# fbcotter/pytorch_wavelets

Measured on AMD Instinct MI355X. Metric: Mpixels/s fwd+inv DWT J=3 db4, Nx3x512x512 fp32; % HBM roofline, higher is better.
Workload: dtype f32; 1 GPU; DWTForward+DWTInverse J=3 db4 symmetric, 128x3x512x512 fp32 per GPU (BASELINE configs[1]); global_batch=128, parallelism=batch-sharded x1, no data-path collective, step=forward + inverse

## Files before the change

### pytorch_wavelets_amd/csrc/wl_api.inc

```
#include "../../include/wavelets_hip.h"
#include "wl_common.h"
#include "wl_api_common.h"
#include "wl_dt_api.h"
#include <string.h>
#include "wl_dwt_kernels.h"
#include "wl_dwt_tile.h"
#include "wl_dwt_tile_syn.h"
#include "wl_dwt_direct.h"
#include "wl_nonsep.h"
#include "wl_dwt_small.h"
#include "wl_filt1d.h"
#include "wl_swt2d.h"
#include "wl_iswt2d.h"
#include "wl_dwt3d.h"
#include "wl_dtcwt_kernels.h"
#include "wl_dtcwt_tile.h"
#include "wl_dtcwt_rot.h"
#include "wl_dtcwt_small.h"

template <typename T>
struct WlAfb2dTile {
    typedef WlAfb2dArgs<T> Args;
    static const int kThreads = 256;
    static const int kMinWaves = 1;
    static WL_DEV void run(const Args& a, const WlCtx& ctx) { wl_afb2d_tile_body<T>(a, ctx); }
};
template <typename T>
struct WlSfb2dTile {
    typedef WlSfb2dArgs<T> Args;
    static const int kThreads = 256;
    static const int kMinWaves = 1;
    static WL_DEV void run(const Args& a, const WlCtx& ctx) { wl_sfb2d_tile_body<T>(a, ctx); }
};

extern "C" int wl_version(void) { return 220; }
extern "C" const char* wl_backend(void) { return WL_BACKEND_NAME; }
extern "C" int wl_dwt_coeff_len(int n, int L, int mode) { return wl_coeff_len(n, L, mode); }

struct WlOptions {
    int generic_only;
    int no_stream;
    int scat_stream;
    WlOptions() {
        const char* v = getenv("WL_GENERIC_ONLY");
        generic_only = (v && *v) ? atoi(v) : 0;
        no_stream = 0;
        scat_stream = 0;
    }
};
static WlOptions& wl_options() { static WlOptions o; return o; }
extern "C" int wl_set_option(const char* name, int value) {
    if (!name) return WL_ERR_SHAPE;
    if (!strcmp(name, "generic_only")) { wl_options().generic_only = value; return 0; }
    if (!strcmp(name, "no_stream")) { wl_options().no_stream = value; return 0; }
    if (!strcmp(name, "scat_stream")) { wl_options().scat_stream = value; return 0; }
    return WL_ERR_UNSUPPORTED;
}
extern "C" int wl_get_option(const char* name) {
    if (!name) return WL_ERR_SHAPE;
    if (!strcmp(name, "generic_only")) return wl_options().generic_only;
    if (!strcmp(name, "no_stream")) return wl_options().no_stream;
    if (!strcmp(name, "scat_stream")) return wl_options().scat_stream;
    return WL_ERR_UNSUPPORTED;
}
extern "C" const char* wl_last_kernel(void) { return wl_last_kernel_name(); }
extern "C" const char* wl_kernel_history(int back) { return wl_kernel_history_name(back); }
extern "C" long long wl_launch_count(void) { return wl_launch_count_value(); }
extern "C" long long wl_last_grid(void) { return wl_last_grid_value(); }
int wl_streaming_off() { return wl_options().no_stream || wl_options().generic_only; }

template <typename T>
static int wl_afb2d_generic(const WlAfbReq& r) {
    typedef typename WlAcc<T>::type A;
    const int H = r.H, W = r.W, Lw = r.Lw, Lh = r.Lh, mode = r.mode;
    WlAfb2dArgs<T> a;
    a.x = (const T*)r.x; a.ll = (T*)r.ll; a.highs = (T*)r.highs;
    a.h_w_lo = (const A*)r.taps.w_lo; a.h_w_hi = (const A*)r.taps.w_hi; a.h_h_lo = (const A*)r.taps.h_lo; a.h_h_hi = (const A*)r.taps.h_hi;
    a.NC = r.planes; a.H = H; a.W = W;
    a.x_ps = r.x_ps; a.ll_ps = r.ll_ps; a.x_rs = r.x_rs; a.ll_rs = r.ll_rs;
    a.Kh = wl_dwt_coeff_len(H, Lh, mode); a.Kw = wl_dwt_coeff_len(W, Lw, mode);
    a.Lw = Lw; a.Lh = Lh;
    a.basew = wl_afb_base(W, Lw, mode); a.baseh = wl_afb_base(H, Lh, mode);
    a.extw = a.exth = wl_mode_to_ext(mode);
    int TH = 16, TW = 64;
    if (a.Kw <= 32) TW = 32;
    if (a.Kh <= 8) TH = 8;
    for (;;) {
        a.TH = TH; a.TW = TW;
        a.nrows = 2 * TH + Lh - 2; a.ncols = 2 * TW + Lw - 2;
        a.spitch = a.ncols | 1;
        if (wl_afb2d_tile_lds(a) <= 64 * 1024 || (TH <= 4 && TW <= 16)) break;
        if (TW > 16) TW /= 2; else TH /= 2;
    }
    a.tiles_x = wl_cdiv(a.Kw, TW); a.tiles_y = wl_cdiv(a.Kh, TH);
    return wl_launch<WlAfb2dTile<T> >(a, r.planes * a.tiles_x * a.tiles_y, wl_afb2d_tile_lds(a), r.stream);
}


template <typename T, int LT, int TH = 16, int TW = 64, int SH = 0, int V4 = 0>
static int wl_afb_tile_launch(const WlAfbReq& r) {
    typedef WlAfbTile<T, LT, TH, TW, SH, V4> K;
    const int64_t planes = r.planes;
// ... 1013 lines not shown
```

### pytorch_wavelets_amd/csrc/wl_api_common.h

```cpp
#pragma once
#include <stdlib.h>
#include "../../include/wavelets_hip.h"
#include "wl_common.h"
#include "wl_lattice.h"

static int wl_mode_to_ext(int mode) {
    switch (mode) {
        case 0: return WL_EXT_ZERO;
        case 1: return WL_EXT_SYM;
        case 2: return WL_EXT_PER;
        case 4: return WL_EXT_REFL;
        case 6: return WL_EXT_PERIODIC;
        default: return -1;
    }
}

static inline int wl_coeff_len(int n, int L, int mode) { return mode == 2 ? (n + 1) / 2 : (n + L - 1) / 2; }

static int wl_afb_base(int n, int L, int mode) {
    if (mode == 2) return L / 2 - L + 1;
    const int K = (n + L - 1) / 2;
    const int p = 2 * (K - 1) - n + L;
    return -(p / 2);
}

struct WlBanks { const void* w_lo; const void* w_hi; const void* h_lo; const void* h_hi; };
struct WlAfbReq {
    const void* x; int64_t x_ps; int x_rs;
    void* ll; int64_t ll_ps; int ll_rs; void* highs;
    int64_t planes; int H, W;
    WlBanks taps; int Lw, Lh, mode;
    int policy; float* scratch; int* tstate; void* stream;
};
struct WlSfbReq {
    const void* ll; int64_t ll_ps; int ll_rs; const void* highs; void* y;
    int64_t planes; int Kh, Kw, OH, OW;
    WlBanks taps; int Lw, Lh, mode;
// ... 61 lines not shown
```

### pytorch_wavelets_amd/csrc/wl_dwt_rows.h

```cpp
#pragma once
#include "wl_common.h"

#define WL_ROWS_MAXLEV 3
#ifndef WL_ROWS_WAVES
#define WL_ROWS_WAVES 12
#endif
#ifndef WL_ROWS_LOADERS
#define WL_ROWS_LOADERS 2
#endif
#define WL_ROWS_MAXHB 768
#ifndef WL_ROWS_ABLATE
#define WL_ROWS_ABLATE 0
#endif
#if (WL_ROWS_ABLATE & 8) && defined(__HIPCC__)
#define WL_TICK() __builtin_readcyclecounter()
#else
#define WL_TICK() 0ull
#endif
#ifndef WL_ROWS_DEPTH
#define WL_ROWS_DEPTH 3
#endif

#if defined(__HIPCC__)
WL_DEV void wl_pk_fma_x(wl_v2& acc, wl_v2 tap, wl_v2 s) {
// ... 33 lines not shown
    int nwaves;
    unsigned ring_magic;
    int ring_rows;
};

struct WlRowsSeg {
    int nhb;
    int f0[WL_ROWS_MAXLEV];
    int fend[WL_ROWS_MAXLEV];
    int own_lo[WL_ROWS_MAXLEV];
    int own_hi[WL_ROWS_MAXLEV];
    unsigned sched[WL_ROWS_MAXHB / 4];
};

template <typename T>
struct WlRowsArgs {
    const T* x;
    T* ll;
    T* yh[WL_ROWS_MAXLEV];
    const float* h_w_lo;
    const float* h_w_hi;
    const float* h_h_lo;
    const float* h_h_hi;
    int64_t NC, x_ps, ll_ps;
    int x_rs, ll_rs;
    int nlev, ext, base;
    int nwhole;
    int zero_off;
    int lds_bytes;
    signed char role_level[WL_ROWS_WAVES];
    short role_col0[WL_ROWS_WAVES];
    signed char role_sub[WL_ROWS_WAVES];
    int pp, lds_plane;
    WlRowsLevel g[WL_ROWS_MAXLEV];
    WlRowsSeg seg[3];
    int guard;
    const float* lat;
};

struct WlRowsSched {
    int fed[WL_ROWS_MAXLEV];
    WL_HD void init(const WlRowsSeg& sg) { for (int j = 0; j < WL_ROWS_MAXLEV; ++j) fed[j] = sg.f0[j]; }
    static WL_HD int src_row(int e, int Hs, int ext) { return ext == WL_EXT_PER ? e : wl_ext1(e, Hs, ext); }
    WL_HD int avail(const WlRowsSeg& sg, int j, int LT) const {
        const int warm = (LT - 2) / 2;
        return fed[j] - sg.f0[j] > warm ? fed[j] - warm : sg.f0[j];
    }
    template <typename A> WL_HD int feeds_now(const A& a, const WlRowsSeg& sg, int j, int LT) const {
        const int left = sg.fend[j] - fed[j];
        if (j == 0) return left > 2 ? 2 : left;
        const int av = avail(sg, j - 1, LT);
        const int Hs = a.g[j].Hs;
        const int e = a.base + 2 * fed[j];
        const bool ok0 = left > 0 && src_row(e, Hs, a.ext) < av && src_row(e + 1, Hs, a.ext) < av;
        const bool ok1 = left > 1 && src_row(e + 2, Hs, a.ext) < av && src_row(e + 3, Hs, a.ext) < av;
        return ok0 ? (ok1 ? 2 : 1) : 0;
    }
};

#ifndef WL_ROWS_SAME_MIN
#define WL_ROWS_SAME_MIN 10
#endif
WL_HD int wl_ring_slot(int r, int rows, unsigned magic) {
    const unsigned u = (unsigned)(r + (rows << 6));
    const unsigned q = (unsigned)(((unsigned long long)u * magic) >> 32);
    const int sl = (int)(u - q * (unsigned)rows);
// ... 8 lines not shown
    static const int kThreads = 64 * WL_ROWS_WAVES;
    static const int kMinWaves = 6;
    static const int LROWS = 4 / WL_ROWS_LOADERS;
    static const int NL = LROWS * PPR;
    static const int WARM = (LT - 2) / 2;
    static const int NSLOT = D + 1;
    static const int SZ = (int)sizeof(T);
    static_assert((D - 1) * NL < 64, "prefetch distance exceeds the vmcnt range");

    static WL_DEV void loader(const Args& a, const WlRowsSeg& sg, const WlCtx& ctx, int64_t plane, int lane, int lidx) {
        const WlRowsLevel& g = a.g[0];
        const char* xp = reinterpret_cast<const char*>(a.x + (size_t)plane * a.x_ps);
        const int row_bytes = g.Ws * SZ;
        const int row_stride = a.x_rs * SZ;
        const int nhb0 = (sg.fend[0] - sg.f0[0] + 1) / 2;
        const int e_last = a.base + 2 * sg.fend[0] - 1;
        const int ring = g.ring_off, pitch = g.ring_pitch, pad = g.pad, Hs = g.Hs, ext = a.ext;
        const int base = a.base + 2 * sg.f0[0];
        const int rfirst = lidx * LROWS;
        const int NH = g.hl + g.hr;
        int hdst[2], hsrc[2];
#pragma unroll
        for (int u = 0; u < 2; ++u) {
            const int it = lane + 64 * u;
            hdst[u] = hsrc[u] = -1;
            if ((ext != WL_EXT_ZERO || row_bytes % 16 != 0) && it < LROWS * NH) {
                const int r = rfirst + it / NH, c = it % NH;
                const int e = c < g.hl ? c - g.hl : g.Ws + (c - g.hl);
                const int s = wl_ext(e, g.Ws, ext);
                hdst[u] = r * pitch + pad + e * SZ;
                hsrc[u] = s < 0 ? -1 : r * pitch + pad + s * SZ;
            }
        }
        auto issue = [&](int h) {
            const int slot = ring + (h % NSLOT) * 4 * pitch + pad;
#pragma unroll
            for (int rr = 0; rr < LROWS; ++rr) {
                const int r = rfirst + rr;
                int e = base + 4 * h + r;
                e = e < e_last ? e : e_last;
                int src = e;
                if ((unsigned)e >= (unsigned)Hs) {
                    src = wl_ext(e, Hs, ext);
                    src = src < 0 ? 0 : src;
                }
                const char* grow = xp + (size_t)src * row_stride;
#pragma unroll
                for (int p = 0; p < PPR; ++p) {
                    const int byte = (p * 64 + lane) * 16;
                    if (!(WL_ROWS_ABLATE & 2)) wl_dma16(ctx, (unsigned)(slot + r * pitch + p * 1024), grow + byte, byte < row_bytes);
                }
            }
        };
        for (int h = 0; h < D; ++h) issue(h);
        unsigned long long tw = 0, tb = 0, ti = 0;
        for (int hb = 0; hb < sg.nhb; ++hb) {
            const unsigned long long c0 = WL_TICK();
            if (hb < nhb0) {
                if (!(WL_ROWS_ABLATE & 2)) wl_wait_vm<(D - 1) * NL>();
                char* slot = ctx.smem + ring + (hb % NSLOT) * 4 * pitch;
#pragma unroll
                for (int u = 0; u < 2; ++u)
                    if (hdst[u] >= 0) *reinterpret_cast<T*>(slot + hdst[u]) = hsrc[u] < 0 ? (T)0 : *reinterpret_cast<const T*>(slot + hsrc[u]);
            }
            const unsigned long long c1 = WL_TICK();
            ctx.sync();
            const unsigned long long c2 = WL_TICK();
            if (hb < nhb0) issue(hb + D);
            const unsigned long long c3 = WL_TICK();
            tw += c1 - c0; tb += c2 - c1; ti += c3 - c2;
        }
        wl_wait_vm<0>();
        if ((WL_ROWS_ABLATE & 8) && lane == 0) {
            T* o = a.ll + (size_t)plane * a.ll_ps;
            o[8] = (T)(float)(tw >> 6); o[9] = (T)(float)(tb >> 6); o[10] = (T)(float)(ti >> 6);
        }
    }

    struct Lane {
        wl_v2 win[LAT ? (KL > 1 ? KL - 1 : 1) : LT];
        unsigned ob;
        int off;
        int ndst, hx0, hx1;
    };
    struct Role {
        wl_v2 tw[LAT ? KL : LT], th[SAME ? 1 : LT];
        wl_v2 lt[LAT ? KL : 1];
        WL_DEV wl_v2 colt(int t) const { return SAME ? tw[LAT ? 0 : t] : th[SAME ? 0 : t]; }
        char* hp0; char* hp1; char* hp2; char* llp;
        unsigned rowb, llrowb, kb;
        int nring, npitch, rmask;
        unsigned nmagic;
        bool last, halo;
    };

    static WL_DEV void load_rows(const Lane& L, const char* smem, int row0, int row1, wl_v2 (&s0)[NP], wl_v2 (&s1)[NP]) {
        const char* p0 = smem + (row0 + L.off);
        const char* p1 = smem + (row1 + L.off);
        if (SZ == 4) {
#pragma unroll
            for (int u = 0; u < NP; ++u) {
// ... 189 lines not shown
        R.llp = reinterpret_cast<char*>(a.ll + (size_t)plane * a.ll_ps);
        R.rowb = (unsigned)g.Kw * SZ; R.llrowb = (unsigned)a.ll_rs * SZ; R.kb = (unsigned)k * SZ;
        const WlRowsLevel& gn = a.g[j + 1 < WL_ROWS_MAXLEV ? j + 1 : j];
        R.nring = gn.ring_off; R.npitch = gn.ring_pitch;
        R.rmask = NP2 ? gn.ring_rows : gn.ring_rows - 1;
        R.nmagic = gn.ring_magic;
        Lane L;
#pragma unroll
        for (int t = 0; t < (LAT ? (KL > 1 ? KL - 1 : 1) : LT); ++t) L.win[t] = wl_v2{0.f, 0.f};
        L.ob = (unsigned)sg.f0[j] * R.rowb + (unsigned)k * SZ;
        L.off = g.pad + (2 * (active ? k : 0) + a.base - ODD) * SZ;
        L.ndst = gn.pad + k * SZ; L.hx0 = L.hx1 = -1;
        if (!R.last && active && a.ext != WL_EXT_ZERO) {
            for (int c = 0; c < gn.hl + gn.hr; ++c) {
                const int e = c < gn.hl ? c - gn.hl : gn.Ws + (c - gn.hl);
                if (wl_ext(e, gn.Ws, a.ext) == k) {
                    if (e < 0) L.hx0 = gn.pad + e * SZ; else L.hx1 = gn.pad + e * SZ;
                }
            }
        }
        R.halo = !R.last && a.ext != WL_EXT_ZERO && (col0 <= gn.hl + 1 || col0 + 63 >= gn.Ws - gn.hr - 2);
        if (R.last) main_loop<j, true, false>(a, sg, ctx, plane, L, R, active, k);
        else if (R.halo) main_loop<j, false, true>(a, sg, ctx, plane, L, R, active, k);
        else main_loop<j, false, false>(a, sg, ctx, plane, L, R, active, k);
    }

    template <int j, bool LAST, bool HALO>
    static WL_DEV void main_loop(const Args& a, const WlRowsSeg& sg, const WlCtx& ctx, int64_t plane, Lane& L, const Role& R,
                                 bool active, int k) {
        const WlRowsLevel& g = a.g[j];
        char* const smem = ctx.smem;
        const int rmask = NP2 ? g.ring_rows : g.ring_rows - 1, zrow = a.zero_off, ring = g.ring_off, pitch = g.ring_pitch, Hs = g.Hs;
        const bool zmode = a.ext == WL_EXT_ZERO, per = a.ext == WL_EXT_PER;
        auto rows_of = [&](int f, int hb, int i, int& r0, int& r1) {
            const int e = a.base + 2 * f;
            if (j == 0) {
                r0 = ring + ((hb % NSLOT) * 4 + 2 * i) * pitch;
                r1 = r0 + pitch;
                if (zmode) {
                    if ((unsigned)e >= (unsigned)Hs) r0 = zrow;
                    if ((unsigned)(e + 1) >= (unsigned)Hs) r1 = zrow;
                }
            } else {
                int s0 = e, s1 = e + 1;
                if (!per && (e < 0 || e + 1 >= Hs)) { s0 = wl_ext1(e, Hs, a.ext); s1 = wl_ext1(e + 1, Hs, a.ext); }
                r0 = zmode && s0 < 0 ? zrow : ring + (NP2 ? wl_ring_slot(s0, rmask, g.ring_magic) : (s0 & rmask)) * pitch;
                r1 = zmode && s1 < 0 ? zrow : ring + (NP2 ? wl_ring_slot(s1, rmask, g.ring_magic) : (s1 & rmask)) * pitch;
            }
            r0 = wl_uniform(r0); r1 = wl_uniform(r1);
        };

        const int f0 = sg.f0[j], own_lo = sg.own_lo[j], own_hi = sg.own_hi[j];
        int fed = f0;
        unsigned long long tb = 0, tf = 0, ts = 0, c3 = WL_TICK();
        for (int hb = 0; hb < sg.nhb; ++hb) {
            const unsigned long long c0 = WL_TICK();
            ts += c0 - c3;
            const int n = wl_uniform((int)(sg.sched[hb >> 2] >> (8 * (hb & 3) + 2 * j)) & 3);
            ctx.sync();
            const unsigned long long c1 = WL_TICK();
            tb += c1 - c0;
            const int orow = fed - WARM;
#ifndef WL_ROWS_FEED2_MAXL
#define WL_ROWS_FEED2_MAXL 10
#endif
            if (LT <= WL_ROWS_FEED2_MAXL && n == 2 && fed - f0 >= WARM) {
                int r0, r1, r2, r3;
                rows_of(fed, hb, 0, r0, r1);
                rows_of(fed + 1, hb, 1, r2, r3);
                if (active)
                    feed2<LAST, HALO>(L, R, smem, r0, r1, r2, r3, orow, orow >= own_lo && orow < own_hi,
                                      orow + 1 >= own_lo && orow + 1 < own_hi);
                fed += 2;
            } else {
                for (int i = 0; i < n; ++i) {
                    int r0, r1;
                    rows_of(fed, hb, i, r0, r1);
                    const int o = fed - WARM;
                    if (active) feed1<LAST, HALO>(L, R, smem, r0, r1, fed - f0 >= WARM, o, o >= own_lo && o < own_hi);
                    ++fed;
                }
            }
            c3 = WL_TICK();
            tf += c3 - c1;
        }
        if ((WL_ROWS_ABLATE & 8) && j == 0 && k == 64) {
            T* o = a.ll + (size_t)plane * a.ll_ps;
            o[0] = (T)(float)(tb >> 6); o[1] = (T)(float)(tf >> 6); o[2] = (T)(float)(ts >> 6);
        }
    }

    static WL_DEV void run(const Args& a, const WlCtx& ctx) {
        const int tid = ctx.tid;
        const int wave = wl_uniform(tid >> 6), lane = tid & 63;
        if (a.guard) {
            const bool holds = a.lat ? *reinterpret_cast<const unsigned*>(a.lat) == WL_LAT_OK
                                     : wl_taps_same(a.h_w_lo, a.h_h_lo, LT) && wl_taps_same(a.h_w_hi, a.h_h_hi, LT);
            if (!wl_guard_pass(a.guard, holds)) return;
        }
        const int64_t bid = ctx.bid;
        const int sub = wl_uniform(a.role_sub[wave]);
        const int64_t plane = (bid < a.nwhole ? bid : a.nwhole + (bid - a.nwhole) / 2) * a.pp + sub;
        const WlRowsSeg& sg = a.seg[bid < a.nwhole ? 0 : 1 + (int)((bid - a.nwhole) & 1)];
        for (int i = tid * 16; i < a.lds_bytes; i += kThreads * 16) {
            wl_f4 z; z.x = z.y = z.z = z.w = 0.f;
            *reinterpret_cast<wl_f4*>(ctx.smem + i) = z;
        }
        ctx.sync();
        WlCtx cs = ctx;
        cs.smem += sub * a.lds_plane; cs.lds_base += (unsigned)(sub * a.lds_plane);
        const int lev = plane < a.NC ? wl_uniform(a.role_level[wave]) : -2, col0 = wl_uniform(a.role_col0[wave]);
        if (lev == -1) loader(a, sg, cs, plane, lane, col0);
        else if (lev == 0) compute<0>(a, sg, cs, plane, col0, lane);
        else if (lev == 1) compute<1>(a, sg, cs, plane, col0, lane);
// ... 6 lines not shown
```

### pytorch_wavelets_amd/csrc/wl_rows_api.inc

```
#include "wl_api_common.h"
#include "wl_dwt_rows.h"

#ifndef WL_ROWS_PACK_CUT
#define WL_ROWS_PACK_CUT 1
#endif
static int wl_rows_pack_and_cut(int64_t planes, int pp_cap, int lds_plane, int rows, int halo, int64_t cost_now, int64_t max_wgs) {
    if (!WL_ROWS_PACK_CUT) return 0;
    const int64_t cus = wl_num_cus(), slots = 2 * cus;
    int p2 = pp_cap < planes ? pp_cap : (int)planes;
    while (p2 > 1 && (p2 * lds_plane > 80 * 1024 || 8 * ((planes + p2 - 1) / p2) < 3 * cus)) --p2;
    if (p2 <= 1) return 0;
    const int64_t wgs = 2 * ((planes + p2 - 1) / p2);
    if (wgs > max_wgs) return 0;
    const int64_t cost = ((wgs + slots - 1) / slots) * (rows / 2 + halo + 8);
    return cost * 10 < cost_now * 9 ? p2 : 0;
}

#if !defined(WL_ROWS_UNIT_SYNTHESIS)
template <typename T>
static int wl_rows_plan_segment(const WlRowsArgs<T>& a, WlRowsSeg& sg, int LT, int* need) {
    const int nlev = a.nlev;
    WlRowsSched sc;
    sc.init(sg);
    for (int j = 0; j < WL_ROWS_MAXLEV; ++j) need[j] = 0;
// ... 9 lines not shown
        if (!any) return WL_ERR_UNSUPPORTED;
        for (int j = 0; j + 1 < nlev; ++j) {
            const int wr_hi = sc.avail(sg, j, LT) + nn[j];
            const int e_next = a.base + 2 * sc.fed[j + 1];
            const int e_last = a.base + 2 * sg.fend[j + 1] - 1;
            int oldest = a.g[j + 1].Hs;
            if (a.ext == WL_EXT_PER) oldest = e_next <= e_last ? e_next : 0x3fffffff;
            else if (e_next <= e_last) {
                const int cand[4] = {e_next, e_last, e_next < 0 ? -1 : e_next, e_next < 0 ? 0 : e_next};
                for (int c = 0; c < 4; ++c) {
                    if (cand[c] < e_next || cand[c] > e_last) continue;
                    const int r = wl_ext1(cand[c], a.g[j + 1].Hs, a.ext);
                    if (r >= 0 && r < oldest) oldest = r;
                }
            }
            if (wr_hi - oldest > need[j + 1]) need[j + 1] = wr_hi - oldest;
        }
        for (int j = 0; j < nlev; ++j) sc.fed[j] += nn[j];
    }
    sg.nhb = nhb;
    return 0;
}

#if defined(__HIPCC__)
#define WL_DECLINE(n) WL_ERR_UNSUPPORTED
#else
#include <stdio.h>
static int wl_decline_trace(int n, int line) {
    if (getenv("WL_EMU_TRACE")) fprintf(stderr, "[wl] fused analysis declined at check %d (wl_rows_api.inc:%d)\n", n, line);
    return WL_ERR_UNSUPPORTED;
}
#define WL_DECLINE(n) wl_decline_trace(n, __LINE__)
#endif
template <typename T, int LT, int PPR, int SAME = 0, int LAT = 0, int ODD = 0, int NP2 = 0>
static int wl_afb_rows_launch(const WlAfbPyrReq& r, const float* lat, int guard = 0, int what = 0) {
    typedef WlAfbRows<T, LT, PPR, WL_ROWS_DEPTH, SAME, LAT, ODD, NP2> K;
    const int WARM = (LT - 2) / 2;
    const int64_t planes = r.planes;
    const int H = r.H, W = r.W, nlev = r.nlev, mode = r.mode, strips = r.strips;
    WlRowsArgs<T> a;
    a.ext = wl_mode_to_ext(mode);
    const bool per = a.ext == WL_EXT_PER;
    if (nlev < 1 || nlev > WL_ROWS_MAXLEV) return WL_DECLINE(1);
    if (nlev > 1 && !(a.ext == WL_EXT_ZERO || a.ext == WL_EXT_SYM || a.ext == WL_EXT_REFL || per)) return WL_DECLINE(2);
    if ((int64_t)H * r.x_rs >= (1LL << 30) || r.x_rs < W) return WL_DECLINE(3);
    if ((r.x_rs * sizeof(T)) % 16 != 0 || (r.x_ps * sizeof(T)) % 16 != 0 || (uintptr_t)r.x % 16 != 0 || wl_cdiv(W * (int)sizeof(T), 1024) != PPR) return WL_DECLINE(4);
    if ((W * sizeof(T)) % 16 != 0 && wl_align_up(W * (int)sizeof(T), 16) > r.x_rs * (int)sizeof(T)) return WL_DECLINE(5);
    a.base = wl_afb_base(W, LT, mode);
    if ((a.base & 1) != ODD) return WL_DECLINE(6);
    a.nlev = nlev;
    int compute_waves = 0;
    {
        int h = H, w = W, wave = 0;
        for (int j = 0; j < nlev; ++j) {
            WlRowsLevel& g = a.g[j];
            g.Hs = h; g.Ws = w;
            if (per && (h + (h & 1) < LT - 1 || w + (w & 1) < LT - 1)) return WL_DECLINE(7);
            g.Kh = wl_coeff_len(h, LT, mode); g.Kw = wl_coeff_len(w, LT, mode);
            g.nwaves = wl_cdiv(g.Kw, 64); wave += g.nwaves;
            g.hl = (a.base < 0 ? -a.base : 0) + ODD;
            const int e_max = 2 * (g.Kw - 1) + a.base + LT - 1 + ODD;
            g.hr = e_max > w - 1 ? e_max - (w - 1) : 0;
            if (g.hl > w || g.hr > w || (4 / WL_ROWS_LOADERS) * (g.hl + g.hr) > 128) return WL_DECLINE(8);
            g.pad = wl_align_up(g.hl * (int)sizeof(T), 16);
            g.ring_pitch = wl_align_up(g.pad + (w + g.hr) * (int)sizeof(T), 16);
            if (j > 0) {
// ... 46 lines not shown
        if (NP2) r0 = 2;
        for (int j = 0; j < WL_ROWS_MAXLEV; ++j) a.g[j].ring_rows = r0;
    }
    for (;;) {
        bool bad = false;
        for (int t = 0; t < (can_split ? 3 : 1) && !bad; ++t) {
            int need[WL_ROWS_MAXLEV];
            const int rc = wl_rows_plan_segment<T>(a, a.seg[t], LT, need);
            if (rc) { if (t == 0) return rc; can_split = false; break; }
            for (int j = 1; j < nlev; ++j)
                if (need[j] > a.g[j].ring_rows) {
                    if (NP2) a.g[j].ring_rows = need[j];
                    else a.g[j].ring_rows *= 2;
                    bad = true;
                    if (a.g[j].ring_rows > 64) return WL_DECLINE(13);
                }
        }
        if (!bad) break;
    }
    for (int j = 0; j < WL_ROWS_MAXLEV; ++j) a.g[j].ring_magic = (unsigned)(0x100000000ull / (unsigned)a.g[j].ring_rows);
    if (NP2)
        for (int j = 1; j < nlev; ++j) {
            const int rows = a.g[j].ring_rows, hi = a.g[j].Hs + 2 * LT + rows;
            int lo = a.base < 0 ? a.base : 0;
            if (-a.g[j].hl < lo) lo = -a.g[j].hl;
            if (-a.g[j - 1].hl < lo) lo = -a.g[j - 1].hl;
            unsigned long long seen = 0;
            for (int r = lo; r < lo + rows; ++r) seen |= 1ull << wl_ring_slot(r, rows, a.g[j].ring_magic);
            if (seen != (rows == 64 ? ~0ull : (1ull << rows) - 1)) return WL_DECLINE(16);
            for (int r = lo; r + rows <= hi; ++r)
                if (wl_ring_slot(r + rows, rows, a.g[j].ring_magic) != wl_ring_slot(r, rows, a.g[j].ring_magic)) return WL_DECLINE(16);
        }
    if (strips == 2 && !can_split) return WL_DECLINE(14);
    {
        int zero_bytes = 0;
        off = 0;
        for (int j = 0; j < nlev; ++j) {
            a.g[j].ring_off = off;
            off += (j == 0 ? 4 * K::NSLOT : a.g[j].ring_rows) * a.g[j].ring_pitch;
            if (a.g[j].ring_pitch > zero_bytes) zero_bytes = a.g[j].ring_pitch;
        }
        for (int j = nlev; j < WL_ROWS_MAXLEV; ++j) a.g[j].ring_off = a.g[nlev - 1].ring_off;
        a.zero_off = off; off += zero_bytes;
#if !defined(__HIPCC__)
        if (off > 80 * 1024 && getenv("WL_EMU_TRACE"))
            for (int j = 0; j < nlev; ++j) fprintf(stderr, "[wl]   level %d: ring rows %d pitch %d\n", j, j == 0 ? 4 * K::NSLOT : a.g[j].ring_rows, a.g[j].ring_pitch);
#endif
        if constexpr (!NP2 && !ODD && LT >= 12 && ((SAME && LAT) || (!SAME && !LAT))) {
            if (off > 80 * 1024 && nlev > 1)
                return wl_afb_rows_launch<T, LT, PPR, SAME, LAT, ODD, 1>(r, lat, guard, what);
        }
        if (off > 80 * 1024) return WL_DECLINE(15);
    }
    const int pp_cap = WL_ROWS_WAVES / (compute_waves + WL_ROWS_LOADERS);
    int pp = pp_cap;
    a.lds_plane = wl_align_up(off, 16);
    while (pp > 1 && (pp * a.lds_plane > 80 * 1024 || (planes + pp - 1) / pp < (int64_t)wl_num_cus())) --pp;
    if (strips == 2) pp = 1;
    bool pack_cut = false;
    if (strips == 0 && can_split && pp == 1 && pp_cap > 1) {
        const int64_t slots = 2 * (int64_t)wl_num_cus();
        const int p2 = wl_rows_pack_and_cut(planes, pp_cap, a.lds_plane, a.g[0].Kh, WARM, ((planes + slots - 1) / slots) * (int64_t)(a.g[0].Kh + 8), wl_num_cus());
        if (p2) { pp = p2; pack_cut = true; }
    }
    a.pp = pp;
    if (pp > 1) off = pp * a.lds_plane;
    a.lds_bytes = off;
    const int64_t units = (planes + pp - 1) / pp;
    int64_t ncut = 0;
    if (can_split && strips == 2) ncut = planes;
    else if (pack_cut) ncut = units;
    else if (can_split && strips == 0 && pp == 1) {
        const int64_t cus = wl_num_cus(), slots = 2 * cus;
        const int64_t rounds = (planes + slots - 1) / slots;
        ncut = rounds * slots - planes;
        if (ncut > planes) ncut = planes;
        if (rounds > 1 && ncut * 4 > planes) ncut = 0;
        if (planes <= cus) ncut = cus - planes < planes ? cus - planes : planes;
    }
    a.nwhole = (int)(units - ncut);
    {
        int load[4] = {0, 0, 0, 0}, cnt[4] = {0, 0, 0, 0};
        const int cap[4] = {(WL_ROWS_WAVES + 3) / 4, (WL_ROWS_WAVES + 2) / 4, (WL_ROWS_WAVES + 1) / 4, WL_ROWS_WAVES / 4};
        for (int w = 0; w < WL_ROWS_WAVES; ++w) { a.role_level[w] = -2; a.role_col0[w] = 0; a.role_sub[w] = 0; }
        int sub = 0;
        auto place = [&](int level, int col0, int cost) {
            int best = -1;
            for (int b = 0; b < 4; ++b)
                if (cnt[b] < cap[b] && (best < 0 || load[b] < load[best])) best = b;
            const int w = best + 4 * cnt[best];
            a.role_level[w] = (signed char)level; a.role_col0[w] = (short)col0; a.role_sub[w] = (signed char)sub;
            load[best] += cost; ++cnt[best];
        };
        for (sub = 0; sub < pp; ++sub)
            for (int j = 0; j < nlev; ++j)
                for (int c = 0; c < a.g[j].nwaves; ++c) place(j, 64 * c, 8 >> j);
        for (sub = 0; sub < pp; ++sub)
            for (int l = 0; l < WL_ROWS_LOADERS; ++l) place(-1, l, 4 / WL_ROWS_LOADERS);
    }
    a.x = (const T*)r.x; a.ll = (T*)r.yl;
    for (int j = 0; j < nlev; ++j) a.yh[j] = (T*)r.yh[j];
    a.h_w_lo = (const float*)r.taps.w_lo; a.h_w_hi = (const float*)r.taps.w_hi;
    a.h_h_lo = (const float*)r.taps.h_lo; a.h_h_hi = (const float*)r.taps.h_hi;
    a.NC = planes; a.x_ps = r.x_ps; a.x_rs = r.x_rs;
    a.ll_ps = (int64_t)a.g[nlev - 1].Kh * a.g[nlev - 1].Kw; a.ll_rs = a.g[nlev - 1].Kw;
    a.guard = guard;
    a.lat = lat;
    if (what == 1) return 0;
    return what == 2 ? wl_launch_armed<K>(a, units + ncut, (size_t)off, r.stream) : wl_launch<K>(a, units + ncut, (size_t)off, r.stream);
}

#ifndef WL_ROWS_LAT_MIN
#define WL_ROWS_LAT_MIN 10
#endif
template <typename T, int LT, int PPR, int ODD = 0>
static int wl_afb_rows_pick(const WlAfbPyrReq& r) {
    const bool same_hint = (r.hints & 1) != 0, qmf_hint = (r.hints & 2) != 0;
    const float* const none = nullptr;
    if constexpr (LT >= WL_ROWS_LAT_MIN) {
        if (same_hint && qmf_hint && r.scratch)
            return wl_lattice_launch<LT>([&](int guard, int what) { return wl_afb_rows_launch<T, LT, PPR, 0, 0, ODD>(r, r.scratch, guard, what); },
                                         [&](int guard, int what) { return wl_afb_rows_launch<T, LT, PPR, 1, 1, ODD>(r, r.scratch, guard, what); },
                                         r.taps, 0, 1, sizeof(T), r.scratch, r.tstate, 3, r.stream);
    }
    if constexpr (LT > 12) return WL_ERR_UNSUPPORTED;
    else {
        if constexpr (LT >= WL_ROWS_SAME_MIN && !ODD) {
            if (r.taps.w_lo == r.taps.h_lo && r.taps.w_hi == r.taps.h_hi) return wl_afb_rows_launch<T, LT, PPR, 1>(r, none);
            if (same_hint) WL_GUARDED_PAIR((wl_afb_rows_launch<T, LT, PPR, 1>), (wl_afb_rows_launch<T, LT, PPR, 0>), r, none);
        }
        return wl_afb_rows_launch<T, LT, PPR, 0, 0, ODD>(r, none);
    }
}

template <typename T>
static int wl_afb_rows_dispatch(const WlAfbPyrReq& r) {
    const int ppr = wl_cdiv(r.W * (int)sizeof(T), 1024);
    const bool odd = (wl_afb_base(r.W, r.L, r.mode) & 1) != 0;
#define WL_PICK(LT_, P_)                                                               \
    do {                                                                               \
        if constexpr (LT_ % 4 == 0) { if (odd) return wl_afb_rows_pick<T, LT_, P_, 1>(r); } \
// ... 35 lines not shown
}

extern "C" int wl_dwt2d_analysis_fused(const void* x, void* yl, void* const* yh, int dtype, int64_t planes,
                                       int H, int W, int nlev, const void* h_w_lo, const void* h_w_hi,
                                       const void* h_h_lo, const void* h_h_hi, int L, int mode, int strips, void* stream) {
    return wl_dwt2d_analysis_fused_ex(x, (int64_t)H * W, W, yl, yh, dtype, planes, H, W, nlev, h_w_lo, h_w_hi, h_h_lo, h_h_hi,
                                      L, mode, strips, nullptr, nullptr, stream);
}


#endif

#if !defined(WL_ROWS_UNIT_ANALYSIS)
#include "wl_idwt_rows.h"

template <typename T>
static int wl_irows_plan_segment(const WlIRowsArgs<T>& a, WlIRowsSeg& sg, int LT) {
    WlIRowsSched sc;
    sc.init(sg);
    int nhb = 0;
    for (;; ++nhb) {
        int nn[WL_IROWS_MAXLEV], todo = 0, any = 0;
        for (int j = 0; j < a.nlev; ++j) { nn[j] = sc.feeds_now(a, sg, j, LT); todo += sg.fend[j] - sc.fed[j]; any += nn[j]; }
        if (todo == 0) break;
        if (nhb >= WL_IROWS_MAXHB || !any) return WL_ERR_UNSUPPORTED;
        if ((nhb & 3) == 0) sg.sched[nhb >> 2] = 0;
        for (int j = 0; j < a.nlev; ++j) sg.sched[nhb >> 2] |= (unsigned)nn[j] << (8 * (nhb & 3) + 2 * j);
        for (int j = 0; j < a.nlev; ++j) sc.fed[j] += nn[j];
    }
    sg.nhb = nhb;
    return 0;
}

template <typename T, int LT, int LAT = 0, int PER = 0>
static int wl_sfb_rows_launch(const WlSfbPyrReq& r, const float* lat = nullptr, int guard = 0, int what = 0) {
    typedef WlSfbRows<T, LT, LAT, PER> K;
    const int SZ = (int)sizeof(T), WARM = K::WARM;
    const int64_t planes = r.planes, ll_ps = r.yl_ps;
    const int ll_rs = r.yl_rs, yl_h = r.yl_h, yl_w = r.yl_w, nlev = r.nlev, strips = r.strips;
    const void* const yl = r.yl; const void* const* const yh = r.yh;
    const int* const Kh = r.Kh; const int* const Kw = r.Kw;
    WlIRowsArgs<T> a;
    if (nlev < 1 || nlev > WL_IROWS_MAXLEV) return WL_ERR_UNSUPPORTED;
    a.nlev = nlev;
    a.per = PER;
    int compute_waves = 0;
    {
        int sh = yl_h, sw = yl_w;
        for (int j = nlev - 1; j >= 0; --j) {
            WlIRowsLevel& g = a.g[j];
            g.Kh = Kh[j]; g.Kw = Kw[j];
            if (g.Kh < LT / 2 || g.Kw < LT / 2) return WL_ERR_UNSUPPORTED;
            if (sh < g.Kh || sh > g.Kh + 1 || sw < g.Kw || sw > g.Kw + 1) return WL_ERR_SHAPE;
            if (PER && (sh != g.Kh || sw != g.Kw)) return WL_ERR_UNSUPPORTED;
            g.OH = PER ? 2 * g.Kh : 2 * g.Kh - LT + 2; g.OW = PER ? 2 * g.Kw : 2 * g.Kw - LT + 2;
            g.per_d0 = 0; g.head_off = -1;
            if ((int64_t)g.Kh * g.Kw >= (1LL << 28)) return WL_ERR_UNSUPPORTED;
            g.rbytes = g.Kw * SZ;
            if (g.rbytes % 4 != 0 || ((int64_t)g.Kh * g.rbytes) % 4 != 0 || (uintptr_t)yh[j] % 4 != 0) return WL_ERR_UNSUPPORTED;
#ifndef WL_IROWS_R0
#define WL_IROWS_R0 8
#endif
            g.dma_rows = j == 0 ? WL_IROWS_R0 : 8; g.dma_shift = j == 0 && WL_IROWS_R0 == 16 ? 4 : 3;
            if (PER) {
                g.per_d0 = wl_align_up(WARM * SZ, 16);
                g.rbytes = wl_align_up(g.per_d0 + g.Kw * SZ, 16);
// ... 49 lines not shown
    const int OH0 = a.g[0].OH;
    int M = (OH0 / 2) & ~1;
    if (PER) M &= ~((2 << nlev) - 1);
    bool can_split = M >= 2 && M + 2 <= OH0;
    for (int t = 0; t < 3; ++t)
        for (int j = 0; j < WL_IROWS_MAXLEV; ++j) a.seg[t].rho[j] = 0;
    for (int t = 0; t < (can_split ? 3 : 1); ++t) {
        WlIRowsSeg& sg = a.seg[t];
        sg.own_lo = t == 2 ? M : 0;
        sg.own_hi = t == 1 ? M : OH0;
        if (PER) {
            const int len = sg.own_hi - sg.own_lo;
            for (int j = 0; j < nlev; ++j) sg.rho[j] = (sg.own_lo / 2) >> j;
            sg.own_lo = 0; sg.own_hi = len;
            sg.f0[0] = 0;
            sg.fend[0] = len / 2 + WARM;
            for (int j = 1; j < nlev; ++j) {
                sg.f0[j] = 0;
                int rows = sg.fend[j - 1];
                if (rows > a.g[j - 1].Kh) rows = a.g[j - 1].Kh;
                sg.fend[j] = (rows + 1) / 2 + WARM;
            }
            continue;
        }
        sg.f0[0] = sg.own_lo / 2;
        sg.fend[0] = (sg.own_hi + 1) / 2 + WARM;
        if (sg.fend[0] > a.g[0].Kh) sg.fend[0] = a.g[0].Kh;
        for (int j = 1; j < nlev; ++j) {
            sg.f0[j] = sg.f0[j - 1] / 2;
            sg.fend[j] = (sg.fend[j - 1] - 1) / 2 + WARM + 1;
            if (sg.fend[j] > a.g[j].Kh) sg.fend[j] = a.g[j].Kh;
        }
    }
    int off = 0;
    for (int rr = 4;; rr *= 2) {
        off = 0;
        for (int j = 0; j < nlev; ++j) {
            WlIRowsLevel& g = a.g[j];
            if (j + 1 < nlev) {
                int cols = g.Kw;
                if (2 * wl_cdiv(a.g[j + 1].OW, 2) > cols) cols = 2 * wl_cdiv(a.g[j + 1].OW, 2);
                if (PER) cols += WARM;
                g.ll_rows = rr; g.ll_pitch = wl_align_up(cols * SZ, 16);
            } else { g.ll_rows = g.dma_rows; g.ll_pitch = g.rbytes; }
            for (int s = 0; s < 4; ++s) {
                g.src_off[s] = off;
                off += s == 0 ? g.ll_rows * g.ll_pitch : wl_align_up(g.dma_rows * g.rbytes, 16);
                if (PER && s == 0 && j + 1 < nlev) { g.head_off = off; off += (WARM > 0 ? WARM : 1) * g.ll_pitch; }
            }
        }
        bool ok = true;
        for (int t = 0; t < (can_split ? 3 : 1); ++t) {
            const int rc = wl_irows_plan_segment<T>(a, a.seg[t], LT);
            if (rc) { if (t == 0) return rc; can_split = false; break; }
            WlIRowsArgs<T> b = a;
            for (int j = 0; j < nlev; ++j) b.g[j].ll_rows = 1 << 20;
            wl_irows_plan_segment<T>(b, b.seg[t], LT);
            if (a.seg[t].nhb > b.seg[t].nhb + 2) ok = false;
        }
        if (ok || nlev == 1) break;
        if (rr >= 64) return WL_ERR_UNSUPPORTED;
    }
    for (int j = nlev; j < WL_IROWS_MAXLEV; ++j) { a.g[j] = a.g[nlev - 1]; a.g[j].nwaves = 0; a.yh[j] = nullptr; }
    if (off > 80 * 1024) return WL_ERR_UNSUPPORTED;
    int pp = pp_waves;
    a.lds_plane = wl_align_up(off, 16);
    while (pp > 1 && (pp * a.lds_plane > 80 * 1024 || (planes + pp - 1) / pp < (int64_t)wl_num_cus())) --pp;
    if (strips == 2) pp = 1;
    bool pack_cut = false;
    if (strips == 0 && can_split && pp == 1 && pp_waves > 1) {
        const int64_t slots = 2 * (int64_t)wl_num_cus();
        const int64_t r1 = (planes + slots - 1) / slots;
        const bool halves = r1 == 1 && r1 * slots - planes > 0 && planes > wl_num_cus();
        const int64_t cost_now = halves ? ((2 * planes + slots - 1) / slots) * (int64_t)(OH0 / 4 + LT / 2 + 8) : r1 * (int64_t)(OH0 / 2 + 8);
        const int p2 = wl_rows_pack_and_cut(planes, pp_waves, a.lds_plane, OH0 / 2, LT / 2, cost_now, slots);
        if (p2) { pp = p2; pack_cut = true; }
    }
    a.pp = pp;
    if (pp > 1) off = pp * a.lds_plane;
    a.lds_bytes = off;
    {
        int load[4] = {0, 0, 0, 0}, cnt[4] = {0, 0, 0, 0};
        const int cap[4] = {(WL_IROWS_WAVES + 3) / 4, (WL_IROWS_WAVES + 2) / 4, (WL_IROWS_WAVES + 1) / 4, WL_IROWS_WAVES / 4};
        for (int w = 0; w < WL_IROWS_WAVES; ++w) { a.role_level[w] = -2; a.role_arg[w] = 0; a.role_sub[w] = 0; }
        int sub = 0;
        auto place = [&](int level, int arg, int cost) {
            int best = -1;
            for (int b = 0; b < 4; ++b)
                if (cnt[b] < cap[b] && (best < 0 || load[b] < load[best])) best = b;
            const int w = best + 4 * cnt[best];
            a.role_level[w] = (signed char)level; a.role_arg[w] = (short)arg; a.role_sub[w] = (signed char)sub;
            load[best] += cost; ++cnt[best];
        };
        for (sub = 0; sub < pp; ++sub)
            for (int j = 0; j < nlev; ++j)
                for (int c = 0; c < a.g[j].nwaves; ++c) place(j, 64 * c, 16 >> j);
        for (sub = 0; sub < pp; ++sub)
            for (int l = 0; l < nld; ++l) place(-1, ld[l].level * 16 + ld[l].s0 * 4 + (ld[l].ns - 1), ld[l].level == 0 ? 3 : 2);
    }
    if (strips == 2 && !can_split) return WL_ERR_UNSUPPORTED;
    const int64_t units = (planes + pp - 1) / pp;
    int64_t ncut = 0;
    if (can_split && strips == 2) ncut = planes;
    else if (pack_cut) ncut = units;
    else if (can_split && strips == 0 && pp == 1) {
        const int64_t cus = wl_num_cus(), slots = 2 * cus;
        const int64_t rounds = (planes + slots - 1) / slots;
        ncut = rounds * slots - planes;
        if (ncut > planes) ncut = planes;
        if (rounds > 1 && ncut * 4 > planes) ncut = 0;
        if (rounds == 1 && ncut > 0) ncut = planes;
        if (planes <= cus) ncut = cus - planes < planes ? cus - planes : planes;
    }
    a.nwhole = (int)(units - ncut);
    a.yl = (const T*)yl; a.ll_ps = ll_ps;
    for (int j = 0; j < nlev; ++j) a.yh[j] = (const T*)yh[j];
    a.y = (T*)r.y;
    a.g_w_lo = (const float*)r.taps.w_lo; a.g_w_hi = (const float*)r.taps.w_hi;
    a.g_h_lo = (const float*)r.taps.h_lo; a.g_h_hi = (const float*)r.taps.h_hi;
    a.NC = planes;
    a.guard = guard; a.lat = lat;
    if (what == 1) return 0;
    return what == 2 ? wl_launch_armed<K>(a, units + ncut, (size_t)off, r.stream) : wl_launch<K>(a, units + ncut, (size_t)off, r.stream);
}

template <typename T, int LT, int PER = 0>
static int wl_sfb_rows_pick(const WlSfbPyrReq& r) {
    if constexpr (LT >= WL_IROWS_LAT_MIN) {
        if ((r.hints & 3) == 3 && r.scratch)
            return wl_lattice_launch<LT>([&](int guard, int what) { return wl_sfb_rows_launch<T, LT, 0, PER>(r, r.scratch, guard, what); },
                                         [&](int guard, int what) { return wl_sfb_rows_launch<T, LT, 1, PER>(r, r.scratch, guard, what); },
                                         r.taps, 1, 1, sizeof(T), r.scratch, r.tstate, 3, r.stream);
    }
    if constexpr (LT > 12) return WL_ERR_UNSUPPORTED;
    else return wl_sfb_rows_launch<T, LT, 0, PER>(r);
}

template <typename T>
static int wl_sfb_rows_dispatch(const WlSfbPyrReq& r) {
#define WL_CASE(LT_) case LT_: return r.mode == 2 ? wl_sfb_rows_pick<T, LT_, 1>(r) : wl_sfb_rows_pick<T, LT_, 0>(r)
    switch (r.L) {
        WL_CASE(2); WL_CASE(4); WL_CASE(6); WL_CASE(8); WL_CASE(10); WL_CASE(12); WL_CASE(14); WL_CASE(16); WL_CASE(18); WL_CASE(20);
        default: return WL_ERR_UNSUPPORTED;
    }
#undef WL_CASE
}

extern "C" int wl_dwt2d_synthesis_fused_ex(const void* yl, int64_t yl_plane_stride, int yl_row_stride, int yl_h, int yl_w,
                                           const void* const* yh, const int* Kh, const int* Kw, void* y, int dtype,
                                           int64_t planes, int nlev, const void* g_w_lo, const void* g_w_hi,
                                           const void* g_h_lo, const void* g_h_hi, int L, int mode, int strips,
                                           void* tap_scratch, int* tap_state, void* stream) {
    if (wl_mode_to_ext(mode) < 0) return WL_ERR_MODE;
    if (planes < 0 || yl_h < 1 || yl_w < 1) return WL_ERR_SHAPE;
    if (L < 1 || L > WL_MAX_TAPS) return WL_ERR_TAPS;
// ... 21 lines not shown
```

### pytorch_wavelets_amd/ops.py

```python
import contextlib
import ctypes
import threading
import torch

from . import _lib

_DTYPES = {torch.float32: 0, torch.float16: 1, torch.float64: 2, torch.bfloat16: 3}
_TEST_BACKEND = None


def _backend():
    return _TEST_BACKEND if _TEST_BACKEND is not None else _lib.get()


def _check_tensor(t, name):
    if t.dtype not in _DTYPES:
        raise TypeError('%s: unsupported dtype %s (float16/bfloat16/float32/float64)' % (name, t.dtype))
    if not t.is_cuda and _TEST_BACKEND is None:
        raise RuntimeError('%s is on %s: pytorch_wavelets_amd runs on MI355X only (HIP kernels, '
                           'no CPU fallback). Move the module and its input to a cuda device.'
                           % (name, t.device))


class _NoGuard(object):
# ... 233 lines not shown
    return bool(getattr(_HINTS, 'qmf', False)), bool(getattr(_HINTS, 'same', False))


@contextlib.contextmanager
def hints(qmf, same):
    with qmf_hint(qmf), same_banks_hint(same):
        yield


def banks_equal(lo_a, hi_a, lo_b, hi_b):
    f = lambda t: t.detach().reshape(-1).double().cpu()
    return (lo_a.numel() == lo_b.numel() and hi_a.numel() == hi_b.numel() and lo_a.numel() > 0
            and bool(torch.equal(f(lo_a), f(lo_b))) and bool(torch.equal(f(hi_a), f(hi_b))))


@contextlib.contextmanager
def same_banks_hint(flag):
    prev = getattr(_HINTS, 'same', False)
    _HINTS.same = bool(flag)
    try:
        yield
    finally:
        _HINTS.same = prev


STREAM_FORCE = False
FUSED_STRIPS = 0
_FUSED_DECLINED = set()
_FUSED_DECLINED_MAX = 4096


def _remember_decline(key):
    be = _backend()
    if be.wl_get_option(b'generic_only') or be.wl_get_option(b'no_stream') or be.wl_get_option(b'scat_stream'):
        return
    if len(_FUSED_DECLINED) >= _FUSED_DECLINED_MAX:
        _FUSED_DECLINED.clear()
    _FUSED_DECLINED.add(key)


def _declined(key, name, ref, *args, memo=True):
    rc = _call(name, ref, *args)
    if rc == _lib.WL_ERR_UNSUPPORTED:
        if memo:
            _remember_decline(key)
        return True
    _lib.check(rc, name)
    return False


def set_option(name, value):
    _FUSED_DECLINED.clear()
    rc = _backend().wl_set_option(name.encode() if isinstance(name, str) else name, int(value))
    _lib.check(rc, 'wl_set_option')


def _num_cus(device):
    if device.type != 'cuda':
        return 2
    idx = device.index if device.index is not None else torch.cuda.current_device()
    if idx not in _CU_COUNT:
        _CU_COUNT[idx] = torch.cuda.get_device_properties(idx).multi_processor_count
    return _CU_COUNT[idx]


def afb2d_fused(x, h_w_lo, h_w_hi, h_h_lo, h_h_hi, mode, nlev, strips=None, whole=True):
    _check_tensor(x, 'x')
# ... 1000 lines not shown
```

Before: 296,300 Mpixels/s.

## Size row-DMA prefetch depth and inverse DMA rows to fit LDS budget

The forward rows kernel now takes its prefetch ring depth at runtime instead of the compile-time constant. The depth is chosen as the deepest setting (up to a cap) whose LDS layout fits within 80KB, and the wait count and slot indexing become dynamic. The inverse rows kernel likewise doubles each level's DMA row batch up to a cap while the LDS still fits. The aim is more memory loads in flight to hide HBM latency, at the cost of more LDS per block (possibly lower occupancy) and dynamic vmcnt waits.

```diff
diff --git a/pytorch_wavelets_amd/csrc/wl_api.inc b/pytorch_wavelets_amd/csrc/wl_api.inc
--- a/pytorch_wavelets_amd/csrc/wl_api.inc
+++ b/pytorch_wavelets_amd/csrc/wl_api.inc
@@ -41,11 +41,16 @@
     int generic_only;
     int no_stream;
     int scat_stream;
+    int rows_depth;
+    int irows_dma_rows;
+    int rows_depth_last, irows_dma_rows_last;
     WlOptions() {
         const char* v = getenv("WL_GENERIC_ONLY");
         generic_only = (v && *v) ? atoi(v) : 0;
         no_stream = 0;
         scat_stream = 0;
+        rows_depth = irows_dma_rows = 0;
+        rows_depth_last = irows_dma_rows_last = 0;
     }
 };
 static WlOptions& wl_options() { static WlOptions o; return o; }
@@ -54,6 +59,8 @@
     if (!strcmp(name, "generic_only")) { wl_options().generic_only = value; return 0; }
     if (!strcmp(name, "no_stream")) { wl_options().no_stream = value; return 0; }
     if (!strcmp(name, "scat_stream")) { wl_options().scat_stream = value; return 0; }
+    if (!strcmp(name, "rows_depth")) { wl_options().rows_depth = value; return 0; }
+    if (!strcmp(name, "irows_dma_rows")) { wl_options().irows_dma_rows = value; return 0; }
     return WL_ERR_UNSUPPORTED;
 }
 extern "C" int wl_get_option(const char* name) {
@@ -61,6 +68,10 @@
     if (!strcmp(name, "generic_only")) return wl_options().generic_only;
     if (!strcmp(name, "no_stream")) return wl_options().no_stream;
     if (!strcmp(name, "scat_stream")) return wl_options().scat_stream;
+    if (!strcmp(name, "rows_depth")) return wl_options().rows_depth;
+    if (!strcmp(name, "irows_dma_rows")) return wl_options().irows_dma_rows;
+    if (!strcmp(name, "rows_depth_last")) return wl_options().rows_depth_last;
+    if (!strcmp(name, "irows_dma_rows_last")) return wl_options().irows_dma_rows_last;
     return WL_ERR_UNSUPPORTED;
 }
 extern "C" const char* wl_last_kernel(void) { return wl_last_kernel_name(); }
@@ -68,6 +79,10 @@
 extern "C" long long wl_launch_count(void) { return wl_launch_count_value(); }
 extern "C" long long wl_last_grid(void) { return wl_last_grid_value(); }
 int wl_streaming_off() { return wl_options().no_stream || wl_options().generic_only; }
+int wl_rows_depth_option() { return wl_options().rows_depth; }
+int wl_irows_dma_rows_option() { return wl_options().irows_dma_rows; }
+void wl_rows_note_depth(int depth) { wl_options().rows_depth_last = depth; }
+void wl_irows_note_dma_rows(int rows) { wl_options().irows_dma_rows_last = rows; }
 
 template <typename T>
 static int wl_afb2d_generic(const WlAfbReq& r) {
diff --git a/pytorch_wavelets_amd/csrc/wl_api_common.h b/pytorch_wavelets_amd/csrc/wl_api_common.h
--- a/pytorch_wavelets_amd/csrc/wl_api_common.h
+++ b/pytorch_wavelets_amd/csrc/wl_api_common.h
@@ -3,6 +3,11 @@
 #include "../../include/wavelets_hip.h"
 #include "wl_common.h"
 #include "wl_lattice.h"
+
+int wl_rows_depth_option();
+int wl_irows_dma_rows_option();
+void wl_rows_note_depth(int depth);
+void wl_irows_note_dma_rows(int rows);
 
 static int wl_mode_to_ext(int mode) {
     switch (mode) {
diff --git a/pytorch_wavelets_amd/csrc/wl_dwt_rows.h b/pytorch_wavelets_amd/csrc/wl_dwt_rows.h
--- a/pytorch_wavelets_amd/csrc/wl_dwt_rows.h
+++ b/pytorch_wavelets_amd/csrc/wl_dwt_rows.h
@@ -89,6 +89,7 @@
     short role_col0[WL_ROWS_WAVES];
     signed char role_sub[WL_ROWS_WAVES];
     int pp, lds_plane;
+    int depth, nslot;
     WlRowsLevel g[WL_ROWS_MAXLEV];
     WlRowsSeg seg[3];
     int guard;
@@ -163,8 +164,13 @@
                 hsrc[u] = s < 0 ? -1 : r * pitch + pad + s * SZ;
             }
         }
+        const int depth = a.depth, slot_bytes = 4 * pitch, ring_bytes = a.nslot * slot_bytes;
+        const int vm_ahead = (depth - 1) * NL;
+        int islot = 0, wslot = 0;
         auto issue = [&](int h) {
-            const int slot = ring + (h % NSLOT) * 4 * pitch + pad;
+            const int slot = ring + islot + pad;
+            islot += slot_bytes;
+            islot = islot == ring_bytes ? 0 : islot;
 #pragma unroll
             for (int rr = 0; rr < LROWS; ++rr) {
                 const int r = rfirst + rr;
@@ -183,13 +189,15 @@
                 }
             }
         };
-        for (int h = 0; h < D; ++h) issue(h);
+        for (int h = 0; h < depth; ++h) issue(h);
         unsigned long long tw = 0, tb = 0, ti = 0;
         for (int hb = 0; hb < sg.nhb; ++hb) {
             const unsigned long long c0 = WL_TICK();
             if (hb < nhb0) {
-                if (!(WL_ROWS_ABLATE & 2)) wl_wait_vm<(D - 1) * NL>();
-                char* slot = ctx.smem + ring + (hb % NSLOT) * 4 * pitch;
+                if (!(WL_ROWS_ABLATE & 2)) wl_wait_vm_dyn(vm_ahead);
+                char* slot = ctx.smem + ring + wslot;
+                wslot += slot_bytes;
+                wslot = wslot == ring_bytes ? 0 : wslot;
 #pragma unroll
                 for (int u = 0; u < 2; ++u)
                     if (hdst[u] >= 0) *reinterpret_cast<T*>(slot + hdst[u]) = hsrc[u] < 0 ? (T)0 : *reinterpret_cast<const T*>(slot + hsrc[u]);
@@ -197,7 +205,7 @@
             const unsigned long long c1 = WL_TICK();
             ctx.sync();
             const unsigned long long c2 = WL_TICK();
-            if (hb < nhb0) issue(hb + D);
+            if (hb < nhb0) issue(hb + depth);
             const unsigned long long c3 = WL_TICK();
             tw += c1 - c0; tb += c2 - c1; ti += c3 - c2;
         }
@@ -453,10 +461,10 @@
         char* const smem = ctx.smem;
         const int rmask = NP2 ? g.ring_rows : g.ring_rows - 1, zrow = a.zero_off, ring = g.ring_off, pitch = g.ring_pitch, Hs = g.Hs;
         const bool zmode = a.ext == WL_EXT_ZERO, per = a.ext == WL_EXT_PER;
-        auto rows_of = [&](int f, int hb, int i, int& r0, int& r1) {
+        auto rows_of = [&](int f, int sl, int i, int& r0, int& r1) {
             const int e = a.base + 2 * f;
             if (j == 0) {
-                r0 = ring + ((hb % NSLOT) * 4 + 2 * i) * pitch;
+                r0 = ring + sl + 2 * i * pitch;
                 r1 = r0 + pitch;
                 if (zmode) {
                     if ((unsigned)e >= (unsigned)Hs) r0 = zrow;
@@ -473,6 +481,8 @@
 
         const int f0 = sg.f0[j], own_lo = sg.own_lo[j], own_hi = sg.own_hi[j];
         int fed = f0;
+        const int slot_bytes = 4 * pitch, ring_bytes = a.nslot * slot_bytes;
+        int sl = 0;
         unsigned long long tb = 0, tf = 0, ts = 0, c3 = WL_TICK();
         for (int hb = 0; hb < sg.nhb; ++hb) {
             const unsigned long long c0 = WL_TICK();
@@ -487,8 +497,8 @@
 #endif
             if (LT <= WL_ROWS_FEED2_MAXL && n == 2 && fed - f0 >= WARM) {
                 int r0, r1, r2, r3;
-                rows_of(fed, hb, 0, r0, r1);
-                rows_of(fed + 1, hb, 1, r2, r3);
+                rows_of(fed, sl, 0, r0, r1);
+                rows_of(fed + 1, sl, 1, r2, r3);
                 if (active)
                     feed2<LAST, HALO>(L, R, smem, r0, r1, r2, r3, orow, orow >= own_lo && orow < own_hi,
                                       orow + 1 >= own_lo && orow + 1 < own_hi);
@@ -496,11 +506,15 @@
             } else {
                 for (int i = 0; i < n; ++i) {
                     int r0, r1;
-                    rows_of(fed, hb, i, r0, r1);
+                    rows_of(fed, sl, i, r0, r1);
                     const int o = fed - WARM;
                     if (active) feed1<LAST, HALO>(L, R, smem, r0, r1, fed - f0 >= WARM, o, o >= own_lo && o < own_hi);
                     ++fed;
                 }
+            }
+            if (j == 0) {
+                sl += slot_bytes;
+                sl = sl == ring_bytes ? 0 : sl;
             }
             c3 = WL_TICK();
             tf += c3 - c1;
diff --git a/pytorch_wavelets_amd/csrc/wl_rows_api.inc b/pytorch_wavelets_amd/csrc/wl_rows_api.inc
--- a/pytorch_wavelets_amd/csrc/wl_rows_api.inc
+++ b/pytorch_wavelets_amd/csrc/wl_rows_api.inc
@@ -65,6 +65,9 @@
 }
 #define WL_DECLINE(n) wl_decline_trace(n, __LINE__)
 #endif
+#ifndef WL_ROWS_DEPTH_CAP
+#define WL_ROWS_DEPTH_CAP 6
+#endif
 template <typename T, int LT, int PPR, int SAME = 0, int LAT = 0, int ODD = 0, int NP2 = 0>
 static int wl_afb_rows_launch(const WlAfbPyrReq& r, const float* lat, int guard = 0, int what = 0) {
     typedef WlAfbRows<T, LT, PPR, WL_ROWS_DEPTH, SAME, LAT, ODD, NP2> K;
@@ -177,16 +180,19 @@
                 if (wl_ring_slot(r + rows, rows, a.g[j].ring_magic) != wl_ring_slot(r, rows, a.g[j].ring_magic)) return WL_DECLINE(16);
         }
     if (strips == 2 && !can_split) return WL_DECLINE(14);
-    {
-        int zero_bytes = 0;
-        off = 0;
+    auto layout = [&](int nslot) {
+        int zero_bytes = 0, o = 0;
         for (int j = 0; j < nlev; ++j) {
-            a.g[j].ring_off = off;
-            off += (j == 0 ? 4 * K::NSLOT : a.g[j].ring_rows) * a.g[j].ring_pitch;
+            a.g[j].ring_off = o;
+            o += (j == 0 ? 4 * nslot : a.g[j].ring_rows) * a.g[j].ring_pitch;
             if (a.g[j].ring_pitch > zero_bytes) zero_bytes = a.g[j].ring_pitch;
         }
         for (int j = nlev; j < WL_ROWS_MAXLEV; ++j) a.g[j].ring_off = a.g[nlev - 1].ring_off;
-        a.zero_off = off; off += zero_bytes;
+        a.zero_off = o;
+        return o + zero_bytes;
+    };
+    {
+        off = layout(K::NSLOT);
 #if !defined(__HIPCC__)
         if (off > 80 * 1024 && getenv("WL_EMU_TRACE"))
             for (int j = 0; j < nlev; ++j) fprintf(stderr, "[wl]   level %d: ring rows %d pitch %d\n", j, j == 0 ? 4 * K::NSLOT : a.g[j].ring_rows, a.g[j].ring_pitch);
@@ -209,6 +215,25 @@
         if (p2) { pp = p2; pack_cut = true; }
     }
     a.pp = pp;
+    {
+        const int dmin = K::NSLOT - 1;
+        auto fits = [&](int d) {
+            if (d < dmin || (d - 1) * K::NL > WL_IROWS_MAX_VM) return false;
+            const int o = layout(d + 1);
+            return (pp > 1 ? pp * wl_align_up(o, 16) : o) <= 80 * 1024;
+        };
+        const int forced = wl_rows_depth_option();
+        int depth = dmin;
+        if (forced > 0) {
+            if (!fits(forced)) return WL_DECLINE(17);
+            depth = forced;
+        } else
+            for (int d = WL_ROWS_DEPTH_CAP; d > dmin; --d)
+                if (fits(d)) { depth = d; break; }
+        a.depth = depth; a.nslot = depth + 1;
+        off = layout(a.nslot);
+        a.lds_plane = wl_align_up(off, 16);
+    }
     if (pp > 1) off = pp * a.lds_plane;
     a.lds_bytes = off;
     const int64_t units = (planes + pp - 1) / pp;
@@ -252,6 +277,7 @@
     a.guard = guard;
     a.lat = lat;
     if (what == 1) return 0;
+    if (what != 2) wl_rows_note_depth(a.depth);
     return what == 2 ? wl_launch_armed<K>(a, units + ncut, (size_t)off, r.stream) : wl_launch<K>(a, units + ncut, (size_t)off, r.stream);
 }
 
@@ -353,6 +379,9 @@
     return 0;
 }
 
+#ifndef WL_IROWS_DMA_ROWS_CAP
+#define WL_IROWS_DMA_ROWS_CAP 32
+#endif
 template <typename T, int LT, int LAT = 0, int PER = 0>
 static int wl_sfb_rows_launch(const WlSfbPyrReq& r, const float* lat = nullptr, int guard = 0, int what = 0) {
     typedef WlSfbRows<T, LT, LAT, PER> K;
@@ -468,9 +497,9 @@
             if (sg.fend[j] > a.g[j].Kh) sg.fend[j] = a.g[j].Kh;
         }
     }
-    int off = 0;
-    for (int rr = 4;; rr *= 2) {
-        off = 0;
+    int off = 0, ll_rr = 4;
+    auto layout = [&](int rr) {
+        int o = 0;
         for (int j = 0; j < nlev; ++j) {
             WlIRowsLevel& g = a.g[j];
             if (j + 1 < nlev) {
@@ -480,11 +509,16 @@
                 g.ll_rows = rr; g.ll_pitch = wl_align_up(cols * SZ, 16);
             } else { g.ll_rows = g.dma_rows; g.ll_pitch = g.rbytes; }
             for (int s = 0; s < 4; ++s) {
-                g.src_off[s] = off;
-                off += s == 0 ? g.ll_rows * g.ll_pitch : wl_align_up(g.dma_rows * g.rbytes, 16);
-                if (PER && s == 0 && j + 1 < nlev) { g.head_off = off; off += (WARM > 0 ? WARM : 1) * g.ll_pitch; }
+                g.src_off[s] = o;
+                o += s == 0 ? g.ll_rows * g.ll_pitch : wl_align_up(g.dma_rows * g.rbytes, 16);
+                if (PER && s == 0 && j + 1 < nlev) { g.head_off = o; o += (WARM > 0 ? WARM : 1) * g.ll_pitch; }
             }
         }
+        return o;
+    };
+    for (int rr = 4;; rr *= 2) {
+        off = layout(rr);
+        ll_rr = rr;
         bool ok = true;
         for (int t = 0; t < (can_split ? 3 : 1); ++t) {
             const int rc = wl_irows_plan_segment<T>(a, a.seg[t], LT);
@@ -513,6 +547,31 @@
         if (p2) { pp = p2; pack_cut = true; }
     }
     a.pp = pp;
+    if (!PER) {
+        auto fits = [&](int o) { return (pp > 1 ? pp * wl_align_up(o, 16) : o) <= 80 * 1024; };
+        auto resize = [&](int j, int rows) {
+            WlIRowsLevel& g = a.g[j];
+            while (g.dma_rows < rows) { g.dma_rows *= 2; ++g.dma_shift; }
+            while (g.dma_rows > rows) { g.dma_rows /= 2; --g.dma_shift; }
+            g.cpr = wl_cdiv(g.dma_rows * g.rbytes, WL_IROWS_CHUNK);
+        };
+        const int forced = wl_irows_dma_rows_option();
+        if (forced > 0) {
+            if (forced < a.g[0].dma_rows || forced > 32 || (forced & (forced - 1))) return WL_ERR_UNSUPPORTED;
+            resize(0, forced);
+            if (!fits(layout(ll_rr))) return WL_ERR_UNSUPPORTED;
+        } else {
+            for (int j = 0; j < nlev; ++j)
+                while (2 * a.g[j].dma_rows <= WL_IROWS_DMA_ROWS_CAP) {
+                    const int was = a.g[j].dma_rows;
+                    resize(j, 2 * was);
+                    if (!fits(layout(ll_rr))) { resize(j, was); break; }
+                }
+        }
+        off = layout(ll_rr);
+        for (int j = nlev; j < WL_IROWS_MAXLEV; ++j) { const int nw = a.g[j].nwaves; a.g[j] = a.g[nlev - 1]; a.g[j].nwaves = nw; }
+        a.lds_plane = wl_align_up(off, 16);
+    }
     if (pp > 1) off = pp * a.lds_plane;
     a.lds_bytes = off;
     {
@@ -557,6 +616,7 @@
     a.NC = planes;
     a.guard = guard; a.lat = lat;
     if (what == 1) return 0;
+    if (what != 2) wl_irows_note_dma_rows(a.g[0].dma_rows);
     return what == 2 ? wl_launch_armed<K>(a, units + ncut, (size_t)off, r.stream) : wl_launch<K>(a, units + ncut, (size_t)off, r.stream);
 }
 
diff --git a/pytorch_wavelets_amd/ops.py b/pytorch_wavelets_amd/ops.py
--- a/pytorch_wavelets_amd/ops.py
+++ b/pytorch_wavelets_amd/ops.py
@@ -289,7 +289,7 @@
 
 def _remember_decline(key):
     be = _backend()
-    if be.wl_get_option(b'generic_only') or be.wl_get_option(b'no_stream') or be.wl_get_option(b'scat_stream'):
+    if any(be.wl_get_option(o) for o in (b'generic_only', b'no_stream', b'scat_stream', b'rows_depth', b'irows_dma_rows')):
         return
     if len(_FUSED_DECLINED) >= _FUSED_DECLINED_MAX:
         _FUSED_DECLINED.clear()
```

Result: no change. 295,900 Mpixels/s (-0.1%).
